# divortio/divortio-lz4

Measured on NVIDIA B200. Metric: lz4_block_roundtrip_throughput, higher is better.
Workload: dtype u8

## Files before the change

### divortio-lz4_b200/csrc/dlz4_kernels.cuh

```cuda
#pragma once
#include <cuda_runtime.h>
#include <stdint.h>
#include <limits.h>

namespace dlz4 {

#ifdef DLZ4_PHASE_TIMING
__device__ unsigned long long g_phase[16];
#define PT_DECL unsigned long long pt_acc[16] = {0,0,0,0,0,0,0,0,0,0,0,0,0,0,0,0}; long long pt_t = clock64();
#define PT_MARK(i) { const long long pt_n = clock64(); pt_acc[i] += (unsigned long long)(pt_n - pt_t); pt_t = pt_n; }
#define PT_COUNT(i, v) { pt_acc[i] += (v); }
#define PT_FLUSH if (lane_id() == 0) { for (int pt_k = 0; pt_k < 16; ++pt_k) atomicAdd(&g_phase[pt_k], pt_acc[pt_k]); }
#define PT_USE(x) asm volatile("" ::"r"((uint32_t)(x)));
#else
#define PT_DECL
#define PT_MARK(i)
#define PT_COUNT(i, v)
#define PT_FLUSH
#define PT_USE(x)
#endif

#ifndef DLZ4_DEC_MINB
#define DLZ4_DEC_MINB 6
#endif
#ifndef DLZ4_DEC_PREFETCH
#define DLZ4_DEC_PREFETCH 1
#endif
#ifndef DLZ4_DEC_Q
#define DLZ4_DEC_Q 2
#endif
constexpr uint32_t FULL = 0xffffffffu;
constexpr int kHashEntries = 16384;

enum : uint8_t { ST_OK = 0, ST_OUTPUT_TOO_SMALL = 1, ST_MALFORMED = 2, ST_OFFSET_ZERO = 3, ST_DICT_OOB = 4 };

__device__ __forceinline__ uint32_t lane_id() { return threadIdx.x & 31u; }

__device__ __forceinline__ uint32_t ld32u(const uint8_t *p) {
    const uintptr_t a = reinterpret_cast<uintptr_t>(p);
    const uint32_t *w = reinterpret_cast<const uint32_t *>(a & ~static_cast<uintptr_t>(3));
    const uint32_t sh = static_cast<uint32_t>(a & 3u) * 8u;
    const uint32_t lo = w[0];
    if (sh == 0) return lo;
    return __funnelshift_r(lo, w[1], sh);
}

__device__ __forceinline__ void st32u(uint8_t *p, uint32_t v) {
    if ((reinterpret_cast<uintptr_t>(p) & 3u) == 0) { *reinterpret_cast<uint32_t *>(p) = v; return; }
    p[0] = (uint8_t)v; p[1] = (uint8_t)(v >> 8); p[2] = (uint8_t)(v >> 16); p[3] = (uint8_t)(v >> 24);
}

__device__ __forceinline__ void warp_copy(uint8_t *d, const uint8_t *s, uint32_t n, uint32_t lane) {
    if (n <= 64) {
        if (lane < n) d[lane] = s[lane];
        if (lane + 32 < n) d[lane + 32] = s[lane + 32];
        return;
    }
    const uint32_t head = static_cast<uint32_t>(-reinterpret_cast<intptr_t>(d)) & 3u;
    if (lane < head) d[lane] = s[lane];
    d += head; s += head; n -= head;
    const uint32_t nw = n >> 2;
    uint32_t *dw = reinterpret_cast<uint32_t *>(d);
    if ((reinterpret_cast<uintptr_t>(s) & 3u) == 0) {
        const uint32_t *sw = reinterpret_cast<const uint32_t *>(s);
        for (uint32_t i = lane; i < nw; i += 32) dw[i] = sw[i];
    } else {
        for (uint32_t i = lane; i < nw; i += 32) dw[i] = ld32u(s + 4 * i);
    }
    const uint32_t done = nw << 2;
    if (lane < n - done) d[done + lane] = s[done + lane];
}

__device__ __forceinline__ uint32_t skip_sum(uint32_t x) {
    const uint32_t q = x >> 6, r = x & 63u;
    return 32u * q * (q - 1u) + q * r;
}

struct SrcFlat {
    const uint8_t *base;
    __device__ __forceinline__ uint32_t ld32(int32_t v) const { return ld32u(base + v); }
    __device__ __forceinline__ const uint8_t *lit_ptr(int32_t v) const { return base + v; }
};
struct SrcSplit {
    const uint8_t *prefix; int32_t plen; const uint8_t *blk;
    __device__ __forceinline__ uint32_t byte(int32_t v) const { return v < plen ? prefix[v] : blk[v - plen]; }
    __device__ __forceinline__ uint32_t ld32(int32_t v) const {
        if (v >= plen) return ld32u(blk + (v - plen));
        if (v + 4 <= plen) return ld32u(prefix + v);
        return byte(v) | (byte(v + 1) << 8) | (byte(v + 2) << 16) | (byte(v + 3) << 24);
    }
    __device__ __forceinline__ const uint8_t *lit_ptr(int32_t v) const { return blk + (v - plen); }
};

struct Tab16 {
    uint16_t *t; int32_t start;
    __device__ __forceinline__ int32_t get(uint32_t h) const { return start + (int32_t)t[h]; }
    __device__ __forceinline__ void put(uint32_t h, int32_t p) { t[h] = (uint16_t)(p - start); }
};
struct TabG16 {
    uint16_t *t; int32_t start;
    __device__ __forceinline__ int32_t get(uint32_t h) const { return start + (int32_t)__ldcg(t + h); }
    __device__ __forceinline__ void put(uint32_t h, int32_t p) { __stcg(t + h, (uint16_t)(p - start)); }
};
template <bool kGlobal>
struct Tab12e {
    uint16_t *t; int32_t start; uint32_t epoch;
    __device__ __forceinline__ uint32_t ld(uint32_t h) const { return kGlobal ? (uint32_t)__ldcg(t + h) : (uint32_t)t[h]; }
    __device__ __forceinline__ void st(uint32_t h, uint32_t v) { if (kGlobal) __stcg(t + h, (uint16_t)v); else t[h] = (uint16_t)v; }
    __device__ __forceinline__ int32_t dec(uint32_t v) const { return (v >> 12) == epoch ? start + (int32_t)(v & 4095u) : -1; }
    __device__ __forceinline__ int32_t get(uint32_t h) const { return dec(ld(h)); }
    __device__ __forceinline__ void put(uint32_t h, int32_t p) { st(h, (epoch << 12) | (uint32_t)(p - start)); }
};
template <bool kGlobal>
struct TabOv {
    uint16_t *ov; const int32_t *base; int32_t start; uint32_t epoch;
    __device__ __forceinline__ uint32_t raw(uint32_t h) const {
        const uint32_t v = kGlobal ? (uint32_t)__ldcg(ov + h) : (uint32_t)ov[h];
        return (v >> 12) == epoch ? (uint32_t)(start + (int32_t)(v & 4095u) + 1) : (uint32_t)__ldg(base + h);
    }
    __device__ __forceinline__ void st(uint32_t h, uint32_t v) { if (kGlobal) __stcg(ov + h, (uint16_t)v); else ov[h] = (uint16_t)v; }
    __device__ __forceinline__ int32_t get(uint32_t h) const { return (int32_t)raw(h) - 1; }
    __device__ __forceinline__ void put(uint32_t h, int32_t p) { st(h, (epoch << 12) | (uint32_t)(p - start)); }
};
struct Tab32 {
    int32_t *t;
    __device__ __forceinline__ int32_t get(uint32_t h) const { return t[h] - 1; }
    __device__ __forceinline__ void put(uint32_t h, int32_t p) { t[h] = p + 1; }
};

template <class Src>
__device__ __forceinline__ uint8_t *emit_literals(uint8_t *d, const Src &S, int32_t anchor, uint32_t lit,
                                                   uint32_t token_low, uint32_t lane) {
    const uint32_t tok = ((lit < 15u ? lit : 15u) << 4) | token_low;
    if (lane == 0) d[0] = (uint8_t)tok;
    d += 1;
    if (lit >= 15u) {
        const uint32_t rest = lit - 15u, n255 = rest / 255u;
        for (uint32_t i = lane; i < n255; i += 32) d[i] = 255;
        if (lane == 0) d[n255] = (uint8_t)(rest - n255 * 255u);
        d += n255 + 1;
    }
    if (lit) warp_copy(d, S.lit_ptr(anchor), lit, lane);
    return d + lit;
}

template <class Tab, class Src>
__device__ uint32_t compress_block_warp(const Src &S, const int32_t start, const int32_t len, Tab &T, uint8_t *const out) {
    const uint32_t lane = lane_id();
    const uint32_t lt = (1u << lane) - 1u;
    const int32_t sEnd = start + len;
    const int32_t mflimit = sEnd - 12;
    const int32_t matchLimit = sEnd - 5;
    int32_t sIndex = start, anchor = start;
    uint32_t smc = 67;
    uint8_t *d = out;

    while (sIndex < mflimit) {
        const uint32_t base_sum = skip_sum(smc);
        const int32_t p = sIndex + (int32_t)(skip_sum(smc + lane) - base_sum);
        const bool valid = p < mflimit;
        uint32_t seq = 0, h = 0x10000u + lane;
        int32_t cand = -1;
        if (valid) {
            seq = S.ld32(p);
            h = (seq * 2654435761u) >> 18;
            cand = T.get(h);
        }
        const uint32_t same = __match_any_sync(FULL, h);
        const uint32_t prev = same & lt;
        const int j = prev ? 31 - __clz(prev) : (int)lane;
        const int32_t pj = __shfl_sync(FULL, p, j);
        const uint32_t sj = __shfl_sync(FULL, seq, j);
        uint32_t cseq = sj;
        if (prev) cand = pj;
        const bool ok = valid && cand >= 0 && cand != p && (((uint32_t)(p - cand)) >> 16) == 0;
        if (ok && !prev) cseq = S.ld32(cand);
        const bool hit = ok && cseq == seq;
        const uint32_t hits = __ballot_sync(FULL, hit);
        const uint32_t vmask = __ballot_sync(FULL, valid);
        const int hl = __ffs(hits) - 1;
        const uint32_t commit = hits ? ((2u << hl) - 1u) : vmask;
        if (((commit >> lane) & 1u) && ((same & commit) >> lane) == 1u) T.put(h, p);
        __syncwarp();
        if (!hits) {
            if (vmask != FULL) break;
            sIndex += (int32_t)(skip_sum(smc + 32u) - base_sum);
            smc += 32u;
            continue;
        }
        const int32_t s0 = __shfl_sync(FULL, p, hl);
        const int32_t m0 = __shfl_sync(FULL, cand, hl);
        smc = 67;

        int32_t ml;
        for (int32_t base = 4;; base += 128) {
            const int32_t q = s0 + base + 4 * (int32_t)lane;
            int32_t nv = matchLimit - q;
            nv = nv > 4 ? 4 : nv;
            int32_t eq = 0;
            if (nv > 0) {
                const uint32_t x = S.ld32(q) ^ S.ld32(m0 + base + 4 * (int32_t)lane);
                eq = x ? ((__ffs(x) - 1) >> 3) : 4;
                eq = eq < nv ? eq : nv;
            }
            const uint32_t stop = __ballot_sync(FULL, eq < 4);
            if (stop) {
                const int l = __ffs(stop) - 1;
                ml = base + 4 * l + __shfl_sync(FULL, eq, l);
                break;
            }
        }

        const uint32_t code = (uint32_t)(ml - 4);
        d = emit_literals(d, S, anchor, (uint32_t)(s0 - anchor), code < 15u ? code : 15u, lane);
        const uint32_t offset = (uint32_t)(s0 - m0);
        if (lane == 0) { d[0] = (uint8_t)offset; d[1] = (uint8_t)(offset >> 8); }
        d += 2;
        if (code >= 15u) {
            const uint32_t rest = code - 15u, n255 = rest / 255u;
            for (uint32_t i = lane; i < n255; i += 32) d[i] = 255;
            if (lane == 0) d[n255] = (uint8_t)(rest - n255 * 255u);
            d += n255 + 1;
        }
        sIndex = anchor = s0 + ml;
    }
    d = emit_literals(d, S, anchor, (uint32_t)(sEnd - anchor), 0u, lane);
    return (uint32_t)(d - out);
}

struct TabG32 {
    int32_t *t;
    __device__ __forceinline__ int32_t get(uint32_t h) const { return __ldcg(t + h) - 1; }
    __device__ __forceinline__ void put(uint32_t h, int32_t p) { __stcg(t + h, p + 1); }
};

__device__ __forceinline__ uint32_t tab_raw(const Tab16 &T, uint32_t h) { return T.t[h]; }
__device__ __forceinline__ void tab_set_raw(Tab16 &T, uint32_t h, uint32_t v) { T.t[h] = (uint16_t)v; }
__device__ __forceinline__ uint32_t tab_enc(const Tab16 &T, int32_t p) { return (uint32_t)(p - T.start) & 0xFFFFu; }
__device__ __forceinline__ int32_t tab_dec(const Tab16 &T, uint32_t raw) { return T.start + (int32_t)raw; }
__device__ __forceinline__ uint32_t tab_raw(const TabG16 &T, uint32_t h) { return __ldcg(T.t + h); }
__device__ __forceinline__ void tab_set_raw(TabG16 &T, uint32_t h, uint32_t v) { __stcg(T.t + h, (uint16_t)v); }
__device__ __forceinline__ uint32_t tab_enc(const TabG16 &T, int32_t p) { return (uint32_t)(p - T.start) & 0xFFFFu; }
__device__ __forceinline__ int32_t tab_dec(const TabG16 &T, uint32_t raw) { return T.start + (int32_t)raw; }
template <bool G> __device__ __forceinline__ uint32_t tab_raw(const Tab12e<G> &T, uint32_t h) { return T.ld(h); }
template <bool G> __device__ __forceinline__ void tab_set_raw(Tab12e<G> &T, uint32_t h, uint32_t v) { T.st(h, v); }
template <bool G> __device__ __forceinline__ uint32_t tab_enc(const Tab12e<G> &T, int32_t p) { return (T.epoch << 12) | (uint32_t)(p - T.start); }
template <bool G> __device__ __forceinline__ int32_t tab_dec(const Tab12e<G> &T, uint32_t raw) { return T.dec(raw); }
template <bool G> __device__ __forceinline__ uint32_t tab_raw(const TabOv<G> &T, uint32_t h) { return T.raw(h); }
template <bool G> __device__ __forceinline__ void tab_set_raw(TabOv<G> &T, uint32_t h, uint32_t v) { T.st(h, v); }
template <bool G> __device__ __forceinline__ uint32_t tab_enc(const TabOv<G> &T, int32_t p) { return (T.epoch << 12) | (uint32_t)(p - T.start); }
template <bool G> __device__ __forceinline__ int32_t tab_dec(const TabOv<G> &, uint32_t raw) { return (int32_t)raw - 1; }
__device__ __forceinline__ uint32_t tab_raw(const TabG32 &T, uint32_t h) { return (uint32_t)__ldcg(T.t + h); }
__device__ __forceinline__ void tab_set_raw(TabG32 &T, uint32_t h, uint32_t v) { __stcg(T.t + h, (int32_t)v); }
__device__ __forceinline__ uint32_t tab_enc(const TabG32 &, int32_t p) { return (uint32_t)(p + 1); }
__device__ __forceinline__ int32_t tab_dec(const TabG32 &, uint32_t raw) { return (int32_t)raw - 1; }
__device__ __forceinline__ uint32_t tab_raw(const Tab32 &T, uint32_t h) { return (uint32_t)T.t[h]; }
__device__ __forceinline__ void tab_set_raw(Tab32 &T, uint32_t h, uint32_t v) { T.t[h] = (int32_t)v; }
__device__ __forceinline__ uint32_t tab_enc(const Tab32 &, int32_t p) { return (uint32_t)(p + 1); }
__device__ __forceinline__ int32_t tab_dec(const Tab32 &, uint32_t raw) { return (int32_t)raw - 1; }

__device__ __forceinline__ void cp_async4(uint32_t smem_addr, const void *gptr, uint32_t src_size) {
    asm volatile("cp.async.ca.shared.global [%0], [%1], 4, %2;\n" ::"r"(smem_addr), "l"(gptr), "r"(src_size) : "memory");
}
__device__ __forceinline__ void cp_async_commit() { asm volatile("cp.async.commit_group;\n" ::: "memory"); }
template <int N>
__device__ __forceinline__ void cp_async_wait() { asm volatile("cp.async.wait_group %0;\n" ::"n"(N) : "memory"); }

constexpr int kRingLines = 3;
constexpr int kRingBytes = kRingLines * 128;

__device__ __forceinline__ uint32_t ldg_word_guard(const uint8_t *base, int32_t idx, int32_t lo, int32_t hi) {
    return (idx >= lo && idx < hi) ? __ldg(reinterpret_cast<const uint32_t *>(base + idx)) : 0u;
}

struct SpanState {
    int32_t sIndex, anchor;
    uint32_t smc;
    uint32_t D;
    uint32_t pend;
    int32_t head;
};

constexpr uint32_t kSpanStopped = 0xFFFFFFFFu;
template <class Tab, bool kEmit, bool kSplit = false>
__device__ uint32_t compress_span_warp(const uint8_t *__restrict__ base, const int32_t start, const int32_t len, Tab &T,
                                       uint8_t *const out, uint32_t *const ring ,
                                       SpanState &st, const int32_t limit, const uint8_t *__restrict__ pre = nullptr,
                                       const int32_t plen = 0) {
    const uint32_t lane = lane_id();
    const uint32_t lt = (1u << lane) - 1u;
    const int32_t sEnd = start + len;
    const int32_t mflimit = sEnd - 12;
    const int32_t matchLimit = sEnd - 5;
    int32_t sIndex = st.sIndex, anchor = st.anchor;
    uint32_t smc = st.smc;
    uint32_t D = st.D;
    uint32_t pend = st.pend;
    struct SrcSel {
        const uint8_t *base, *pre; int32_t plen;
        __device__ __forceinline__ uint32_t ld32(int32_t v) const {
            if (!kSplit || v >= plen) return ld32u(base + v);
            if (v + 4 <= plen) return ld32u(pre + v);
            uint32_t r = 0;
            for (int k = 0; k < 4; ++k) r |= (uint32_t)(v + k < plen ? pre[v + k] : base[v + k]) << (8 * k);
            return r;
        }
        __device__ __forceinline__ const uint8_t *lit_ptr(int32_t v) const { return base + v; }
    } S{base, pre, plen};

    const uintptr_t gaddr = reinterpret_cast<uintptr_t>(base);
    const int32_t wlo = start - (int32_t)((gaddr + (uint32_t)start) & 3u);
    const int32_t whi = sEnd;
    const uint32_t ring_s = (uint32_t)__cvta_generic_to_shared(ring);
    const uint64_t line0 = (gaddr + (uint32_t)wlo) >> 7;
    uint32_t next_line = 0;
    bool ring_cold = true;
    PT_DECL

    while (sIndex < mflimit) {
        PT_MARK(0)
        if (smc <= 96u && sIndex + 67 <= sEnd && sIndex + 32 <= limit) {
            const int32_t w = sIndex;
            const uint32_t wmis = (uint32_t)((reinterpret_cast<uintptr_t>(base) + (uint32_t)w) & 3u);
            const int32_t wa = w - (int32_t)wmis;
            const uintptr_t waddr = gaddr + (intptr_t)wa;
            const uint32_t L = (uint32_t)((waddr >> 7) - line0);
            if (ring_cold || next_line < L + 3u) {
                if (ring_cold || next_line < L) next_line = L;
                ring_cold = false;
                const bool one_ahead = next_line > L + 1u;
                do {
                    const int32_t idx = wlo - (int32_t)((gaddr + (uint32_t)wlo) & 127u) + (int32_t)(next_line << 7) + 4 * (int32_t)lane;
// ... 477 lines not shown
        for (uint32_t i = lane; i < kVec; i += 32) __stcg(s4 + i, get(i));
        if (lane == 0) snap_state[j] = S;
    }
    const bool last = (J.flags & kSegLast) != 0;
    seg_run<Tab, true>(base, J, block_size, T, ring, S, last ? INT_MAX : J.seg_end, blockbuf, blockbuf_stride, piece_off, piece_len,
                       last ? INT_MAX : J.seg_end);
    if (lane == 0) end_state[j] = S;
    __syncwarp();
    if (kSmem) {
        uint4 *t4 = reinterpret_cast<uint4 *>(tables + (size_t)j * kHashEntries);
        for (uint32_t i = lane; i < kVec; i += 32) __stcg(t4 + i, l4[i]);
        __syncwarp();
    }
}

__device__ __forceinline__ bool seg_differs(const SegState *snap_next, const SegState *end_prev, const int32_t *tab_snap,
                                            const int32_t *tab_end, uint32_t lane) {
    const int2 a = __ldcg(reinterpret_cast<const int2 *>(snap_next)), b = __ldcg(reinterpret_cast<const int2 *>(end_prev));
    int d = (a.x != b.x) | (a.y != b.y);
    const int32_t horizon = b.x - 65535;
    const int4 *A4 = reinterpret_cast<const int4 *>(tab_snap), *B4 = reinterpret_cast<const int4 *>(tab_end);
    auto norm = [&](int32_t v) { v -= 1; return v < horizon ? -1 : v; };
    for (uint32_t i = lane; i < kHashEntries / 4; i += 32) {
        const int4 x = __ldcg(A4 + i), y = __ldcg(B4 + i);
        d |= (norm(x.x) != norm(y.x)) | (norm(x.y) != norm(y.y)) | (norm(x.z) != norm(y.z)) | (norm(x.w) != norm(y.w));
    }
    return __any_sync(FULL, d) != 0;
}

constexpr int kSegWarps = 7;
constexpr int kSegCtasPerSm = 3;
constexpr int kSegSmemBytes = kHashEntries * 4 + kSegWarps * kRingBytes;
__global__ void __launch_bounds__(kSegWarps * 32, kSegCtasPerSm)
k_compress_segments(const uint8_t *__restrict__ base, const SegJob *__restrict__ jobs, const uint32_t *__restrict__ job_list,
                    uint32_t njobs, int32_t block_size, const int32_t *__restrict__ init_table ,
                    int32_t *tables, int32_t *snaps, SegState *snap_state, SegState *end_state,
                    uint8_t *blockbuf, uint64_t blockbuf_stride, uint32_t *piece_off, uint32_t *piece_len, uint32_t *counter,
                    uint32_t active_warps,
                    const uint32_t *landed ,
                    int32_t land_origin, uint32_t land_shift,
                    uint32_t nbig ,
                    uint32_t follow ,
                    const uint8_t *chase_bad ,
                    uint32_t total_jobs, uint32_t *chased ) {
    extern __shared__ __align__(16) uint8_t smem[];
    const uint32_t lane = lane_id(), warp = threadIdx.x >> 5;
    if (warp >= active_warps) return;
    uint32_t *ring = reinterpret_cast<uint32_t *>(smem + kHashEntries * 4 + warp * kRingBytes);
    for (;;) {
        uint32_t q;
        if (nbig) {
            const bool fast = warp == 0;
            const uint32_t n_own = fast ? nbig : njobs - nbig, n_other = njobs - n_own;
            q = next_block(counter + (fast ? 0 : 1), lane);
            if (q < n_own) {
                q += fast ? 0u : nbig;
            } else {
                q = next_block(counter + (fast ? 1 : 0), lane);
                if (q >= n_other) break;
                q += fast ? nbig : 0u;
            }
        } else {
            q = next_block(counter, lane);
            if (q >= njobs) break;
        }
        bool chasing = false;
        for (uint32_t j = job_list ? job_list[q] : q;; ++j) {
            SegJob J = jobs[j];
            if (chasing) J.flags |= kSegRerun;
            if (landed) {
                int32_t need = J.chain_end;
                if (!(J.flags & kSegLast)) {
                    const int32_t be = J.chain_start + (J.seg_end - J.chain_start + block_size - 1) / block_size * block_size;
                    need = be < need ? be : need;
                }
                if (lane == 0) {
                    const volatile uint32_t *f = landed + ((uint32_t)(need - 1 - land_origin) >> land_shift);
                    const long long t0 = clock64();
                    while (*f == 0u) {
                        __nanosleep(500);
                        if (clock64() - t0 > (8ll << 30)) __trap();
                    }
                    __threadfence_system();
                }
                __syncwarp();
            }
            {
                const int32_t last_pos = (J.seg_end < J.chain_end ? J.seg_end : J.chain_end) - 1;
                const uint32_t nslots = (uint32_t)((last_pos - J.chain_start) / block_size - (J.seg_begin - J.chain_start) / block_size) + 1u;
                for (uint32_t i = lane; i < nslots; i += 32) piece_len[J.first_slot + i] = 0;
            }
            if (warp == 0)
                seg_job<Tab32, true>(base, J, j, block_size, init_table, reinterpret_cast<int32_t *>(smem), tables, snaps, snap_state, end_state,
                                     blockbuf, blockbuf_stride, piece_off, piece_len, ring);
            else
                seg_job<TabG32, false>(base, J, j, block_size, init_table, tables + (size_t)j * kHashEntries, tables, snaps, snap_state,
                                       end_state, blockbuf, blockbuf_stride, piece_off, piece_len, ring);
            __syncwarp();
            if (follow) {
                if (!(J.flags & kSegMore)) break;
            } else if (chase_bad) {
                if (j + 1 >= total_jobs || (jobs[j + 1].flags & kSegFirst)) break;
                if (chase_bad[j + 1] && !chase_bad[j]) break;
                if (!seg_differs(snap_state + j + 1, end_state + j, snaps + (size_t)(j + 1) * kHashEntries,
                                 tables + (size_t)j * kHashEntries, lane)) break;
                chasing = true;
                if (lane == 0) atomicAdd(chased, 1u);
            } else {
                break;
            }
        }
    }
}

__global__ void __launch_bounds__(256)
k_seg_verify(const SegJob *__restrict__ jobs, uint32_t njobs, const int32_t *__restrict__ tables, const int32_t *__restrict__ snaps,
             const SegState *__restrict__ snap_state, const SegState *__restrict__ end_state, uint8_t *bad) {
    const uint32_t j = blockIdx.x;
    if (j >= njobs) return;
    __shared__ int diff;
    if (threadIdx.x == 0) diff = 0;
    __syncthreads();
    if (jobs[j].flags & kSegFirst) { if (threadIdx.x == 0) bad[j] = 0; return; }
    const SegState a = snap_state[j], b = end_state[j - 1];
    int d = (a.s != b.s) | (a.head != b.head);
    const int32_t horizon = b.s - 65535;
    const int32_t *ta = snaps + (size_t)j * kHashEntries, *tb = tables + (size_t)(j - 1) * kHashEntries;
    for (uint32_t i = threadIdx.x; i < kHashEntries; i += blockDim.x) {
        int32_t x = ta[i] - 1, y = tb[i] - 1;
        if (x < horizon) x = -1;
        if (y < horizon) y = -1;
        d |= x != y;
    }
    if (d) atomicOr(&diff, 1);
    __syncthreads();
    if (threadIdx.x == 0) bad[j] = (uint8_t)diff;
}

__global__ void __launch_bounds__(256)
k_seg_assemble(const uint8_t *__restrict__ blockbuf, uint64_t blockbuf_stride, const uint32_t *__restrict__ slot_first,
               const uint32_t *__restrict__ slot_count, const uint32_t *__restrict__ piece_off, const uint32_t *__restrict__ piece_len,
               uint32_t nblocks, uint8_t *__restrict__ dst, const uint64_t *__restrict__ dst_off, uint32_t *__restrict__ comp_len) {
    constexpr uint32_t kStripe = 4096;
    for (uint32_t b = blockIdx.x; b < nblocks; b += gridDim.x) {
        const uint8_t *src = blockbuf + (uint64_t)b * blockbuf_stride;
        uint8_t *d = dst + dst_off[b];
        uint32_t pos = 0;
        for (uint32_t k = 0; k < slot_count[b]; ++k) {
            const uint32_t sl = slot_first[b] + k, n = piece_len[sl];
            const uint8_t *s = src + piece_off[sl];
            for (uint32_t st0 = ((pos / kStripe + gridDim.y - 1 - blockIdx.y) / gridDim.y * gridDim.y + blockIdx.y) * kStripe; st0 < pos + n;
                 st0 += gridDim.y * kStripe) {
                const uint32_t lo = st0 > pos ? st0 : pos, hi = st0 + kStripe < pos + n ? st0 + kStripe : pos + n;
                for (uint32_t i = lo + threadIdx.x; i < hi; i += blockDim.x) d[i] = s[i - pos];
            }
            pos += n;
        }
        if (threadIdx.x == 0 && blockIdx.y == 0) comp_len[b] = pos;
    }
}

__global__ void __launch_bounds__(32, 1)
k_compress_chain(const uint8_t *__restrict__ work, int32_t start, int32_t total_len, int32_t block_size, uint32_t nblocks,
                 int32_t *table_io ,
                 uint8_t *__restrict__ dst, uint64_t dst_stride, uint32_t *__restrict__ comp_len) {
    extern __shared__ __align__(16) uint8_t smem[];
    const uint32_t lane = lane_id();
    int32_t *tab = reinterpret_cast<int32_t *>(smem);
    uint4 *t4 = reinterpret_cast<uint4 *>(tab);
    uint4 *g4 = reinterpret_cast<uint4 *>(table_io);
    for (uint32_t i = lane; i < kHashEntries * 4 / 16; i += 32) t4[i] = g4[i];
    __syncwarp();
    Tab32 T{tab};
    const int32_t end = start + total_len;
    for (uint32_t k = 0; k < nblocks; ++k) {
        const int32_t pos = start + (int32_t)k * block_size;
        const int32_t blen = (end - pos) < block_size ? (end - pos) : block_size;
        const uint32_t c = compress_block_warp_v2(work, pos, blen, T, dst + (uint64_t)k * dst_stride,
                                                  reinterpret_cast<uint32_t *>(smem + kHashEntries * 4));
        if (lane == 0) comp_len[k] = c;
        __syncwarp();
    }
    for (uint32_t i = lane; i < kHashEntries * 4 / 16; i += 32) g4[i] = t4[i];
}

__global__ void k_warm_jenkins(const uint8_t *__restrict__ work, int32_t dict_len, int32_t *table) {
    const int32_t i = blockIdx.x * blockDim.x + threadIdx.x;
    if (i > dict_len - 4) return;
    uint32_t h = ld32u(work + i);
    h = h + 2127912214u + (h << 12);
    h = h ^ 3345072700u ^ (h >> 19);
    h = h + 374761393u + (h << 5);
    h = (h + 3550635116u) ^ (h << 9);
    h = h + 4251993797u + (h << 3);
    h = h ^ 3042594569u ^ (h >> 16);
    atomicMax(&table[(h >> 18) & 16383u], i + 1);
}

__device__ __forceinline__ void warp_match_copy(uint8_t *d, uint32_t offset, uint32_t n, uint32_t lane) {
    if (offset >= 32u) {
        const uint8_t *s = d - offset;
        if (offset >= n) { warp_copy(d, s, n, lane); return; }
        for (uint32_t base = 0; base < n; base += 32) {
            const uint32_t k = base + lane;
            if (k < n) d[k] = s[k];
            __syncwarp();
        }
    } else {
        const uint32_t step = 32u - (32u % offset);
        if (lane < step) {
            const uint8_t v = d[(int32_t)(lane % offset) - (int32_t)offset];
            for (uint32_t k = lane; k < n; k += step) d[k] = v;
        }
    }
}

__device__ __forceinline__ bool dec_one_sequence(const uint8_t *__restrict__ in, const uint32_t n, uint8_t *const ob, const uint32_t cap,
                                                 const uint32_t hist, const uint8_t *__restrict__ dict, const uint32_t dict_len,
                                                 uint32_t &ip, uint32_t &op, uint32_t &st, const uint32_t lane) {
    const uint32_t token = in[ip++];
    uint32_t lit = token >> 4;
    if (lit == 15u) {
        uint32_t b;
        do {
            if (ip >= n) { st = ST_MALFORMED; return false; }
            b = in[ip++]; lit += b;
        } while (b == 255u);
    }
    if ((uint64_t)op + lit > cap) { st = ST_OUTPUT_TOO_SMALL; return false; }
    if ((uint64_t)ip + lit > n) { st = ST_MALFORMED; return false; }
    const uint32_t litp = ip;
    ip += lit;
    if (ip >= n) {
        if (lit) warp_copy(ob + op, in + litp, lit, lane);
        op += lit;
        return false;
    }
    if (ip + 2 > n) { if (lit) warp_copy(ob + op, in + litp, lit, lane); st = ST_MALFORMED; return false; }
    const uint32_t offset = (uint32_t)in[ip] | ((uint32_t)in[ip + 1] << 8);
    ip += 2;
    if (offset == 0) { st = ST_OFFSET_ZERO; return false; }
    uint32_t ml = token & 15u;
    if (ml == 15u) {
        uint32_t b;
        do {
            if (ip >= n) { st = ST_MALFORMED; return false; }
            b = in[ip++]; ml += b;
        } while (b == 255u);
    }
    ml += 4;
    const int64_t src_rel = (int64_t)op + lit - offset;
    if (src_rel < -(int64_t)hist) {
        if (lit) warp_copy(ob + op, in + litp, lit, lane);
        op += lit;
        const int64_t cs = src_rel + hist;
        int64_t from_dict = -cs;
        if (from_dict > ml) from_dict = ml;
        const int64_t di = (int64_t)dict_len + cs;
        if (di < 0 || di + from_dict > dict_len) { st = ST_DICT_OOB; return false; }
        if ((uint64_t)op + ml > cap) { st = ST_OUTPUT_TOO_SMALL; return false; }
        warp_copy(ob + op, dict + di, (uint32_t)from_dict, lane);
        op += (uint32_t)from_dict;
        const uint32_t rem = ml - (uint32_t)from_dict;
        __syncwarp();
        if (rem) warp_match_copy(ob + op, offset, rem, lane);
        op += rem;
        __syncwarp();
        return true;
    }
    const uint32_t total = lit + ml;
    if ((uint64_t)op + total > cap) {
        st = ST_OUTPUT_TOO_SMALL;
        return false;
    }
    if (offset >= (total < 32u ? total : 32u)) {
        uint8_t *const d = ob + op;
        const uint8_t *const ls = in + litp;
        const uint8_t *const ms = d - offset;
        for (uint32_t base = 0; base < total; base += 32) {
            const uint32_t j = base + lane;
            if (j < total) d[j] = j < lit ? ls[j] : ms[j];
            __syncwarp();
        }
    } else {
        if (lit) warp_copy(ob + op, in + litp, lit, lane);
        __syncwarp();
        warp_match_copy(ob + op + lit, offset, ml, lane);
        __syncwarp();
    }
    op += total;
    return true;
}

template <bool kDict>
__device__ uint32_t decompress_block_warp_v2(const uint8_t *__restrict__ in, const uint32_t n, uint8_t *const ob,
                                             const uint32_t cap, const uint32_t hist, const uint8_t *__restrict__ dict,
                                             const uint32_t dict_len, uint32_t *status) {
    const uint32_t lane = lane_id();
    uint32_t ip = 0, op = 0;
    uint32_t st = ST_OK;
    while (ip < n) {
        const uint32_t q = ip + lane;
        uint32_t lit = 0, ml = 0, offset = 1, litp = 0, nxt = 1;
        bool stop = true, last = false;
        if (q < n) {
            const uint32_t token = in[q];
            uint32_t p = q + 1;
            lit = token >> 4;
            bool ok = true;
            if (lit == 15u) {
                uint32_t v = 255u;
                for (int k = 0; k < 3 && v == 255u; ++k) {
                    if (p >= n) { ok = false; v = 0; break; }
                    v = in[p++]; lit += v;
                }
                if (v == 255u) ok = false;
            }
            litp = p;
            const uint64_t endlit = (uint64_t)p + lit;
            if (ok && endlit + 2 <= n) {
                offset = (uint32_t)in[endlit] | ((uint32_t)in[endlit + 1] << 8);
                p = (uint32_t)endlit + 2;
                ml = token & 15u;
                if (offset == 0) ok = false;
                else if (ml == 15u) {
                    uint32_t v = 255u;
                    for (int k = 0; k < 3 && v == 255u; ++k) {
                        if (p >= n) { ok = false; v = 0; break; }
                        v = in[p++]; ml += v;
                    }
                    if (v == 255u) ok = false;
                }
                ml += 4;
                nxt = p - ip;
            } else ok = false;
            stop = !ok;
        }
        uint32_t cur = 0, real = 0, myop = 0, opw = op;
        const uint32_t adv = lit + ml;
        const uint32_t stopper = __ballot_sync(FULL, stop);
        while (cur < 32u) {
            if ((stopper >> cur) & 1u) break;
            real |= 1u << cur;
            if (lane == cur) myop = opw;
            opw += __shfl_sync(FULL, adv, cur);
            cur = __shfl_sync(FULL, nxt, cur);
        }
        bool fine = (real >> lane) & 1u;
        uint32_t dsrc = 0;
        if (fine) {
            const int64_t srel = (int64_t)myop + lit - offset;
            if ((uint64_t)myop + lit + ml > cap) fine = false;
            else if (srel < -(int64_t)hist) {
                const int64_t di = (int64_t)dict_len + srel + hist;
                if (kDict && di >= 0 && srel + hist + (int64_t)ml <= 0) dsrc = (uint32_t)di + 1u;
                else fine = false;
            }
#if DLZ4_DEC_PREFETCH
            else asm volatile("prefetch.global.L1 [%0];" ::"l"(ob + srel));
#endif
        }
        const uint32_t notfine = real & ~__ballot_sync(FULL, fine);
        const uint32_t good = notfine ? (real & ((notfine & (0u - notfine)) - 1u)) : real;
        const uint32_t pack = lit | (ml << 16);
        const bool anydict = kDict && __ballot_sync(FULL, dsrc != 0) != 0;
        const uint32_t rel_o = myop - op;
        const bool quick = adv <= 32u && offset >= rel_o + adv && dsrc == 0u;
        if (good && !(good & ~__ballot_sync(FULL, quick))) {
            const uint32_t pa = adv | (lit << 6) | ((litp - ip) << 12) | (rel_o << 18);
            uint8_t *const dw = ob + op + lane;
            const uint8_t *const iw = in + ip + lane;
            uint32_t m = good;
            constexpr int kQ = DLZ4_DEC_Q;
            while (m) {
                const uint8_t *sp[kQ];
                uint8_t *dp[kQ];
                bool pr[kQ];
#pragma unroll
                for (int u = 0; u < kQ; ++u) {
                    const bool valid = m != 0u;
                    const int l = valid ? __ffs(m) - 1 : 0;
                    m &= m - 1u;
                    const uint32_t a = __shfl_sync(FULL, pa, l), of = __shfl_sync(FULL, offset, l);
                    const uint32_t tot = a & 63u, li = (a >> 6) & 63u;
                    pr[u] = valid && lane < tot;
                    dp[u] = dw + (a >> 18);
                    sp[u] = lane < li ? iw + ((a >> 12) & 63u) : dp[u] - of;
                }
                uint8_t v[kQ];
#pragma unroll
                for (int u = 0; u < kQ; ++u) v[u] = pr[u] ? *sp[u] : (uint8_t)0;
#pragma unroll
                for (int u = 0; u < kQ; ++u) if (pr[u]) *dp[u] = v[u];
            }
            __syncwarp();
        } else
        for (uint32_t m = good; m; m &= m - 1u) {
            const int l = __ffs(m) - 1;
            const uint32_t pk = __shfl_sync(FULL, pack, l), off_ = __shfl_sync(FULL, offset, l);
            const uint32_t lp = __shfl_sync(FULL, litp, l), o_ = __shfl_sync(FULL, myop, l);
            const uint32_t lit_ = pk & 0xFFFFu, total = lit_ + (pk >> 16);
            uint8_t *const d = ob + o_;
            if (kDict && anydict) {
                const uint32_t ds = __shfl_sync(FULL, dsrc, l);
                if (ds) {
                    const uint8_t *dsp = dict + (ds - 1u) - lit_;
                    for (uint32_t base = 0; base < total; base += 32) {
                        const uint32_t j = base + lane;
                        if (j < total) d[j] = j < lit_ ? in[lp + j] : dsp[j];
                    }
                    __syncwarp();
                    continue;
                }
            }
            if (off_ >= (total < 32u ? total : 32u)) {
                const uint8_t *sp = lane < lit_ ? in + (lp + lane) : d + ((int32_t)lane - (int32_t)off_);
                uint8_t *dp = d + lane;
                if (total <= 32u) {
                    if (lane < total) *dp = *sp;
                } else {
#pragma unroll 1
                    for (uint32_t base = 0; base < total; base += 32) {
                        const uint32_t j = base + lane;
                        if (j < total) *dp = *sp;
                        dp += 32;
                        sp = j + 32 < lit_ ? in + (lp + j + 32) : d + ((int32_t)(j + 32) - (int32_t)off_);
                        __syncwarp();
                    }
                }
                __syncwarp();
            } else {
                if (lit_) warp_copy(d, in + lp, lit_, lane);
                __syncwarp();
                warp_match_copy(d + lit_, off_, total - lit_, lane);
                __syncwarp();
            }
        }
        if (good) {
            const int hi = 31 - __clz(good);
            op = __shfl_sync(FULL, myop, hi) + __shfl_sync(FULL, adv, hi);
            ip += __shfl_sync(FULL, nxt, hi);
        }
        if (good != real || cur < 32u) {
            if (ip >= n) break;
            if (!dec_one_sequence(in, n, ob, cap, hist, dict, dict_len, ip, op, st, lane)) break;
        }
    }
    *status = st;
    return op;
}

template <int WARPS, bool kDict>
__global__ void __launch_bounds__(WARPS * 32, DLZ4_DEC_MINB)
k_decompress_blocks(const uint8_t *__restrict__ src, const uint64_t *__restrict__ src_off,
                    const uint32_t *__restrict__ src_len, uint32_t nblocks, uint8_t *dst,
                    const uint64_t *__restrict__ dst_off, const uint32_t *__restrict__ dst_cap,
                    const uint8_t *__restrict__ dict, uint32_t dict_len, int hist_frame,
                    const uint8_t *__restrict__ stored ,
                    uint32_t *__restrict__ out_len, uint8_t *__restrict__ status, uint32_t *counter) {
    const uint32_t lane = lane_id();
    const bool twice = !hist_frame && nblocks <= 0x7FFFFFFFu;
    const uint32_t qlen = twice ? 2u * nblocks : nblocks;
    for (;;) {
        const uint32_t qi = next_block(counter, lane);
        if (qi >= qlen) break;
        const uint32_t b = qi < nblocks ? qi : qi - nblocks;
        if (twice) {
            const uint32_t cl = src_len[b], room = dst_cap[b];
            const bool work = !(stored && stored[b]) && cl > (room >> 4) && cl + (room >> 4) < room;
            if (work != (qi < nblocks)) continue;
        }
        uint32_t st;
        uint32_t w;
        if (stored && stored[b]) {
            w = src_len[b];
            st = ST_OK;
            if (w > dst_cap[b]) { st = ST_OUTPUT_TOO_SMALL; w = 0; }
            else warp_copy(dst + dst_off[b], src + src_off[b], w, lane);
        } else {
            const uint64_t o = dst_off[b];
            const uint32_t hist = hist_frame ? (uint32_t)(o < 65536ull ? o : 65536ull) : 0u;
            w = decompress_block_warp_v2<kDict>(src + src_off[b], src_len[b], dst + o, dst_cap[b], hist, dict, dict_len, &st);
        }
        if (lane == 0) { out_len[b] = w; status[b] = (uint8_t)st; }
    }
}

__global__ void __launch_bounds__(32)
k_decompress_chain(const uint8_t *__restrict__ src, const uint64_t *__restrict__ src_off,
                   const uint32_t *__restrict__ src_len, const uint8_t *__restrict__ stored, uint32_t nblocks,
                   uint8_t *dst, uint64_t dst_total, uint32_t block_max, const uint8_t *__restrict__ dict, uint32_t dict_len,
                   uint32_t *__restrict__ out_len, uint8_t *__restrict__ status, uint64_t *total_out) {
    const uint32_t lane = lane_id();
    int64_t op = 0;
    uint32_t st = ST_OK;
    for (uint32_t b = 0; b < nblocks; ++b) {
        uint32_t w = 0;
        if (st == ST_OK) {
            const uint64_t left = dst_total - (uint64_t)op, room = left < block_max ? left : block_max;
            if (stored[b]) {
                w = src_len[b];
                if (w > room) { st = ST_OUTPUT_TOO_SMALL; w = 0; }
                else warp_copy(dst + op, src + src_off[b], w, lane);
                __syncwarp();
            } else {
                w = decompress_block_warp_v2<true>(src + src_off[b], src_len[b], dst + op, (uint32_t)room,
                                             (uint32_t)(op < 65536 ? op : 65536), dict, dict_len, &st);
            }
        }
        if (lane == 0) { out_len[b] = w; status[b] = (uint8_t)st; }
        op += w;
    }
    if (lane == 0) *total_out = (uint64_t)op;
}

struct JdSeq { uint32_t op, ip, lit, ml, off, m0, pad1, pad2; };
constexpr int kJdHopBits = 4;
constexpr int kJdHops = 1 << kJdHopBits;
constexpr uint32_t kJdChunk = 4096;

__device__ __forceinline__ void jd_emit_rec(JdSeq *rec, uint32_t &ns, uint32_t op, uint32_t ip, uint32_t lit, uint32_t ml, uint32_t off,
                                            uint32_t lane) {
    while (lit > kJdChunk) {
        if (lane == 0) rec[ns] = JdSeq{op, ip, kJdChunk, 0u, 0u, 0u, 0u, 0u};
        ++ns; op += kJdChunk; ip += kJdChunk; lit -= kJdChunk;
    }
    uint32_t first = ml > kJdChunk ? kJdChunk : ml;
    const uint32_t m0 = op + lit;
    if (lane == 0) rec[ns] = JdSeq{op, ip, lit, first, off, m0, 0u, 0u};
    ++ns; op += lit + first; ml -= first;
    while (ml) {
        first = ml > kJdChunk ? kJdChunk : ml;
        if (lane == 0) rec[ns] = JdSeq{op, 0u, 0u, first, off, m0, 0u, 0u};
        ++ns; op += first; ml -= first;
    }
}

__device__ __forceinline__ bool jd_scan_one(const uint8_t *__restrict__ in, uint32_t n, uint32_t block_max, JdSeq *rec, uint32_t &ns,
                                            uint32_t &ip, uint64_t &op, uint32_t &rch, uint32_t &st, uint32_t lane) {
    const uint32_t token = in[ip++];
    uint32_t lit = token >> 4;
    if (lit == 15u) {
        uint32_t v;
        do {
            if (ip >= n) { st = ST_MALFORMED; return false; }
            v = in[ip++]; lit += v;
        } while (v == 255u);
    }
    if (op + lit > block_max) { st = ST_OUTPUT_TOO_SMALL; return false; }
    if ((uint64_t)ip + lit > n) { st = ST_MALFORMED; return false; }
    const uint32_t litp = ip;
    ip += lit;
    if (ip >= n) {
        jd_emit_rec(rec, ns, (uint32_t)op, litp, lit, 0u, 0u, lane);
        op += lit;
        return false;
    }
    if (ip + 2 > n) { st = ST_MALFORMED; return false; }
    const uint32_t offset = (uint32_t)in[ip] | ((uint32_t)in[ip + 1] << 8);
    ip += 2;
    if (offset == 0) { st = ST_OFFSET_ZERO; return false; }
    uint32_t ml = token & 15u;
    if (ml == 15u) {
        uint32_t v;
        do {
            if (ip >= n) { st = ST_MALFORMED; return false; }
            v = in[ip++]; ml += v;
        } while (v == 255u);
    }
    ml += 4;
    if (op + lit + ml > block_max) { st = ST_OUTPUT_TOO_SMALL; return false; }
    const int64_t src_rel = (int64_t)op + lit - offset;
    if (src_rel < 0 && (uint32_t)(-src_rel) > rch) rch = (uint32_t)(-src_rel);
    jd_emit_rec(rec, ns, (uint32_t)op, litp, lit, ml, offset, lane);
    op += lit + ml;
    return true;
}

__global__ void __launch_bounds__(128)
k_jd_scan(const uint8_t *__restrict__ src, const uint64_t *__restrict__ src_off, const uint32_t *__restrict__ src_len,
          const uint8_t *__restrict__ stored, uint32_t nblocks, uint32_t block_max, JdSeq *seqs, const uint64_t *__restrict__ seq_base,
          uint32_t *nseq, uint32_t *out_len, uint32_t *reach, uint8_t *status, uint32_t *counter,
          const uint8_t *__restrict__ only ) {
    const uint32_t lane = lane_id();
    const uint32_t lt = (1u << lane) - 1u;
    for (;;) {
        const uint32_t b = next_block(counter, lane);
        if (b >= nblocks) break;
        if (only && !only[b]) continue;
        if (only && lane == 0) reach[b] = 0;
        __syncwarp();
        const uint8_t *in = src + src_off[b];
        const uint32_t n = src_len[b];
        JdSeq *rec = seqs + seq_base[b];
        uint32_t ns = 0, ip = 0, rch = 0, st = ST_OK;
        uint64_t op = 0;
        if (stored[b]) {
            jd_emit_rec(rec, ns, 0u, 0u, n, 0u, 0u, lane);
            op = n;
            if (n > block_max) st = ST_OUTPUT_TOO_SMALL;
        } else {
            while (ip < n) {
                const uint32_t q = ip + lane;
                uint32_t lit = 0, ml = 0, offset = 1, litp = 0, nxt = 1, err = ST_OK;
                bool slow = false, last = false;
                if (q < n) {
                    const uint32_t token = in[q];
                    uint32_t p = q + 1;
                    lit = token >> 4;
                    if (lit == 15u) {
                        uint32_t v = 255u;
                        for (int k = 0; k < 3 && v == 255u; ++k) {
                            if (p >= n) { err = ST_MALFORMED; v = 0; break; }
                            v = in[p++]; lit += v;
                        }
                        if (v == 255u) slow = true;
                    }
                    litp = p;
                    const uint64_t endlit = (uint64_t)p + lit;
                    if (!err && !slow) {
                        if (endlit > n) err = ST_MALFORMED | 0x100u;
                        else if (endlit == n) { last = true; nxt = n - ip; }
                        else if (endlit + 2 > n) err = ST_MALFORMED | 0x200u;
                        else {
                            offset = (uint32_t)in[endlit] | ((uint32_t)in[endlit + 1] << 8);
                            p = (uint32_t)endlit + 2;
                            ml = token & 15u;
                            if (offset == 0) err = ST_OFFSET_ZERO | 0x200u;
                            else if (ml == 15u) {
                                uint32_t v = 255u;
                                for (int k = 0; k < 3 && v == 255u; ++k) {
                                    if (p >= n) { err = ST_MALFORMED | 0x200u; v = 0; break; }
                                    v = in[p++]; ml += v;
                                }
                                if (v == 255u) slow = true;
                            }
                            ml += 4;
                            nxt = p - ip;
                        }
                    }
                    if (lit > kJdChunk || ml > kJdChunk) slow = true;
                }
                uint32_t cur = 0, real = 0, myop = 0;
                uint64_t opw = op;
                const uint32_t adv = lit + ml;
                const uint32_t stopper = __ballot_sync(FULL, slow || err != ST_OK || last || q >= n);
                while (cur < 32u) {
                    real |= 1u << cur;
                    if (lane == cur) myop = (uint32_t)opw;
                    if ((stopper >> cur) & 1u) break;
                    opw += __shfl_sync(FULL, adv, cur);
                    cur = __shfl_sync(FULL, nxt, cur);
                }
                const bool mine = (real >> lane) & 1u;
                uint32_t verdict = ST_OK;
                if (mine && !slow && q < n) {
                    if ((err & 0xFFu) && !(err & 0x300u)) verdict = err;
                    else if ((uint64_t)myop + lit > block_max) verdict = ST_OUTPUT_TOO_SMALL;
                    else if (err) verdict = err & 0xFFu;
                    else if (!last && (uint64_t)myop + lit + ml > block_max) verdict = ST_OUTPUT_TOO_SMALL;
                }
                const uint32_t bad = __ballot_sync(FULL, verdict != ST_OK);
                const uint32_t slowm = __ballot_sync(FULL, mine && (slow || q >= n));
                const uint32_t cut = bad | slowm;
                const uint32_t good = cut ? (real & ((cut & (0u - cut)) - 1u)) : real;
                if ((good >> lane) & 1u) {
                    rec[ns + __popc(good & lt)] = JdSeq{myop, litp, lit, last ? 0u : ml, last ? 0u : offset, myop + lit, 0u, 0u};
                    if (!last) {
                        const int64_t src_rel = (int64_t)myop + lit - offset;
                        if (src_rel < 0) atomicMax(&reach[b], (uint32_t)(-src_rel));
                    }
                }
                ns += __popc(good);
                bool ended = false;
                if (good) {
                    const int hi = 31 - __clz(good);
                    op = (uint64_t)__shfl_sync(FULL, myop, hi) + __shfl_sync(FULL, adv, hi);
                    ip += __shfl_sync(FULL, nxt, hi);
                    ended = __shfl_sync(FULL, (int)last, hi) != 0;
                }
                if (bad && (!slowm || (bad & (0u - bad)) < (slowm & (0u - slowm)))) {
                    st = __shfl_sync(FULL, verdict, __ffs(bad) - 1);
                    break;
                }
                if (ended) break;
                if (slowm && ip < n) {
                    if (!jd_scan_one(in, n, block_max, rec, ns, ip, op, rch, st, lane)) break;
                }
            }
        }
        __syncwarp();
        if (lane == 0) { nseq[b] = ns; out_len[b] = (uint32_t)op; atomicMax(&reach[b], rch); status[b] = (uint8_t)st; }
    }
}

constexpr uint32_t kJdpChunk = 2048;
constexpr uint32_t kJdpSlowBit = 0x80000000u;
struct JdpExit { uint32_t ex, ca; };
struct JdpRun { uint32_t pos, ns, op, pad; };
struct JdpSlow { uint32_t op, litp, lit, ml, off, ns, pad0, pad1; };

__device__ __forceinline__ uint32_t jd_rec_count(uint32_t lit, uint32_t ml) {
    uint32_t c = 1;
    if (lit > kJdChunk) c += (lit - 1) / kJdChunk;
    if (ml > kJdChunk) c += (ml - 1) / kJdChunk;
    return c;
}

__global__ void __launch_bounds__(256)
k_jdp_next(const uint8_t *__restrict__ src, const uint64_t *__restrict__ src_off, const uint32_t *__restrict__ src_len,
           const uint8_t *__restrict__ stored, uint16_t *nx, uint16_t *adv) {
    const uint32_t b = blockIdx.y;
    const uint32_t n = src_len[b];
    const uint32_t i = blockIdx.x * blockDim.x + threadIdx.x;
    if (i >= n || stored[b]) return;
    const uint64_t g = src_off[b];
    const uint8_t *in = src + g;
    const uint32_t token = in[i];
    uint32_t p = i + 1, lit = token >> 4, ml = 0;
    bool ok = true;
    if (lit == 15u) {
        uint32_t v = 255u;
        for (int k = 0; k < 16 && v == 255u; ++k) {
            if (p >= n) { ok = false; v = 0; break; }
            v = in[p++]; lit += v;
        }
        if (v == 255u) ok = false;
    }
    const uint64_t endlit = (uint64_t)p + lit;
    if (ok && endlit + 2 <= n) {
        const uint32_t offset = (uint32_t)in[endlit] | ((uint32_t)in[endlit + 1] << 8);
        p = (uint32_t)endlit + 2;
        ml = token & 15u;
        if (offset == 0) ok = false;
        else if (ml == 15u) {
            uint32_t v = 255u;
            for (int k = 0; k < 16 && v == 255u; ++k) {
                if (p >= n) { ok = false; v = 0; break; }
                v = in[p++]; ml += v;
// ... 613 lines not shown
```

Baseline: 78.58.

## Split warp LZ4 decode into bulk literal scatter and packed match copy

Restructures the per-round decode of the warp-parallel LZ4 decompressor. All literals of the good sequences in a round are now written in one pass, with each lane storing the byte it already loaded at the token position, plus a warp_copy for literals running past 32 bytes. Matches whose sources cannot overlap the round's own output are packed densely across lanes using a prefix sum and ballot-based segment lookup, filling 64 output bytes per iteration instead of one sequence at a time. Remaining matches take a simpler per-sequence path. This targets low lane utilisation on short sequences, at the cost of extra shuffles, scans and reductions per round.

```diff
diff --git a/divortio-lz4_b200/csrc/dlz4_kernels.cuh b/divortio-lz4_b200/csrc/dlz4_kernels.cuh
--- a/divortio-lz4_b200/csrc/dlz4_kernels.cuh
+++ b/divortio-lz4_b200/csrc/dlz4_kernels.cuh
@@ -25,9 +25,6 @@
 #endif
 #ifndef DLZ4_DEC_PREFETCH
 #define DLZ4_DEC_PREFETCH 1
-#endif
-#ifndef DLZ4_DEC_Q
-#define DLZ4_DEC_Q 2
 #endif
 constexpr uint32_t FULL = 0xffffffffu;
 constexpr int kHashEntries = 16384;
@@ -1111,9 +1108,11 @@
     while (ip < n) {
         const uint32_t q = ip + lane;
         uint32_t lit = 0, ml = 0, offset = 1, litp = 0, nxt = 1;
-        bool stop = true, last = false;
+        uint8_t byte = 0;
+        bool stop = true;
         if (q < n) {
             const uint32_t token = in[q];
+            byte = (uint8_t)token;
             uint32_t p = q + 1;
             lit = token >> 4;
             bool ok = true;
@@ -1171,79 +1170,64 @@
         }
         const uint32_t notfine = real & ~__ballot_sync(FULL, fine);
         const uint32_t good = notfine ? (real & ((notfine & (0u - notfine)) - 1u)) : real;
-        const uint32_t pack = lit | (ml << 16);
-        const bool anydict = kDict && __ballot_sync(FULL, dsrc != 0) != 0;
         const uint32_t rel_o = myop - op;
-        const bool quick = adv <= 32u && offset >= rel_o + adv && dsrc == 0u;
-        if (good && !(good & ~__ballot_sync(FULL, quick))) {
-            const uint32_t pa = adv | (lit << 6) | ((litp - ip) << 12) | (rel_o << 18);
+        if (good) {
+            const uint32_t w = __shfl_sync(FULL, (litp - ip) | (lit << 6) | (rel_o << 16), 31 - __clz(good & ((2u << lane) - 1u)));
+            const uint32_t k = lane - (w & 63u);
+            if (k < ((w >> 6) & 1023u)) ob[op + (w >> 16) + k] = byte;
+            const uint32_t wl = __shfl_sync(FULL, w, 31);
+            const uint32_t lp = wl & 63u, le = lp + ((wl >> 6) & 1023u), s0 = lp > 32u ? lp : 32u;
+            if (le > s0) warp_copy(ob + op + (wl >> 16) + (s0 - lp), in + ip + s0, le - s0, lane);
+            __syncwarp();
+        }
+        const uint32_t dense = good & __ballot_sync(FULL, dsrc == 0u && (offset >= rel_o + adv || (ml <= offset && offset <= lit)));
+        if (dense) {
+            uint32_t inc = (dense >> lane) & 1u ? ml : 0u;
+#pragma unroll
+            for (uint32_t d = 1; d < 32u; d <<= 1) {
+                const uint32_t t = __shfl_up_sync(FULL, inc, d);
+                if (lane >= d) inc += t;
+            }
+            const uint32_t mtot = __shfl_sync(FULL, inc, 31);
+            const uint32_t nd = __popc(dense);
+            const int from = lane < nd ? (int)__fns(dense, 0, (int)lane + 1) : 0;
+            const uint32_t mst = __shfl_sync(FULL, inc - ml, from);
+            const uint32_t mp = __shfl_sync(FULL, (rel_o + lit - (inc - ml)) | (offset << 16), from);
+            const uint32_t le = (2u << lane) - 1u;
             uint8_t *const dw = ob + op + lane;
-            const uint8_t *const iw = in + ip + lane;
-            uint32_t m = good;
-            constexpr int kQ = DLZ4_DEC_Q;
-            while (m) {
-                const uint8_t *sp[kQ];
-                uint8_t *dp[kQ];
-                bool pr[kQ];
-#pragma unroll
-                for (int u = 0; u < kQ; ++u) {
-                    const bool valid = m != 0u;
-                    const int l = valid ? __ffs(m) - 1 : 0;
-                    m &= m - 1u;
-                    const uint32_t a = __shfl_sync(FULL, pa, l), of = __shfl_sync(FULL, offset, l);
-                    const uint32_t tot = a & 63u, li = (a >> 6) & 63u;
-                    pr[u] = valid && lane < tot;
-                    dp[u] = dw + (a >> 18);
-                    sp[u] = lane < li ? iw + ((a >> 12) & 63u) : dp[u] - of;
-                }
-                uint8_t v[kQ];
-#pragma unroll
-                for (int u = 0; u < kQ; ++u) v[u] = pr[u] ? *sp[u] : (uint8_t)0;
-#pragma unroll
-                for (int u = 0; u < kQ; ++u) if (pr[u]) *dp[u] = v[u];
+            uint32_t seen = 0;
+            for (uint32_t base = 0; base < mtot; base += 64u) {
+                const uint32_t r0 = mst - base, r1 = r0 - 32u;
+                const uint32_t b0 = __reduce_or_sync(FULL, lane < nd && r0 < 32u ? 1u << r0 : 0u);
+                const uint32_t b1 = __reduce_or_sync(FULL, lane < nd && r1 < 32u ? 1u << r1 : 0u);
+                const uint32_t a0 = __shfl_sync(FULL, mp, seen + __popc(b0 & le) - 1u);
+                seen += __popc(b0);
+                const uint32_t a1 = __shfl_sync(FULL, mp, seen + __popc(b1 & le) - 1u);
+                seen += __popc(b1);
+                uint8_t *const d0 = dw + base + (a0 & 0xFFFFu), *const d1 = dw + base + 32u + (a1 & 0xFFFFu);
+                const bool p0 = base + lane < mtot, p1 = base + 32u + lane < mtot;
+                uint8_t v0 = 0, v1 = 0;
+                if (p0) v0 = d0[-(int32_t)(a0 >> 16)];
+                if (p1) v1 = d1[-(int32_t)(a1 >> 16)];
+                if (p0) *d0 = v0;
+                if (p1) *d1 = v1;
             }
             __syncwarp();
-        } else
-        for (uint32_t m = good; m; m &= m - 1u) {
+        }
+        for (uint32_t m = good & ~dense; m; m &= m - 1u) {
             const int l = __ffs(m) - 1;
-            const uint32_t pk = __shfl_sync(FULL, pack, l), off_ = __shfl_sync(FULL, offset, l);
-            const uint32_t lp = __shfl_sync(FULL, litp, l), o_ = __shfl_sync(FULL, myop, l);
-            const uint32_t lit_ = pk & 0xFFFFu, total = lit_ + (pk >> 16);
-            uint8_t *const d = ob + o_;
-            if (kDict && anydict) {
+            const uint32_t off_ = __shfl_sync(FULL, offset, l), len = __shfl_sync(FULL, ml, l);
+            uint8_t *const d = ob + __shfl_sync(FULL, myop + lit, l);
+            if (kDict) {
                 const uint32_t ds = __shfl_sync(FULL, dsrc, l);
                 if (ds) {
-                    const uint8_t *dsp = dict + (ds - 1u) - lit_;
-                    for (uint32_t base = 0; base < total; base += 32) {
-                        const uint32_t j = base + lane;
-                        if (j < total) d[j] = j < lit_ ? in[lp + j] : dsp[j];
-                    }
+                    warp_copy(d, dict + (ds - 1u), len, lane);
                     __syncwarp();
                     continue;
                 }
             }
-            if (off_ >= (total < 32u ? total : 32u)) {
-                const uint8_t *sp = lane < lit_ ? in + (lp + lane) : d + ((int32_t)lane - (int32_t)off_);
-                uint8_t *dp = d + lane;
-                if (total <= 32u) {
-                    if (lane < total) *dp = *sp;
-                } else {
-#pragma unroll 1
-                    for (uint32_t base = 0; base < total; base += 32) {
-                        const uint32_t j = base + lane;
-                        if (j < total) *dp = *sp;
-                        dp += 32;
-                        sp = j + 32 < lit_ ? in + (lp + j + 32) : d + ((int32_t)(j + 32) - (int32_t)off_);
-                        __syncwarp();
-                    }
-                }
-                __syncwarp();
-            } else {
-                if (lit_) warp_copy(d, in + lp, lit_, lane);
-                __syncwarp();
-                warp_match_copy(d + lit_, off_, total - lit_, lane);
-                __syncwarp();
-            }
+            warp_match_copy(d, off_, len, lane);
+            __syncwarp();
         }
         if (good) {
             const int hi = 31 - __clz(good);
```

After: 79.76 (median of 6 runs). 1.02x the previous value.
